# unslothai/unsloth

Measured on AMD Instinct MI355X. Metric: train tokens/sec, Llama-3-8B QLoRA (NF4) r=16 seq2048 bf16, higher is better.
Workload: dtype bf16; 1 GPU; Llama-3-8B QLoRA NF4 r=16 (q,k,v,o,gate,up,down) seq2048 bf16, fwd+bwd+AdamW; model=Llama-3-8B (synthetic weights), global_batch=4, seq_len=2048, parallelism=dp1, layers=32, lora_rank=16, gradient_checkpointing=unsloth, gc_schedule_chosen=all (every layer keeps everything), nf4_decoded_weight_mirrors=off (every NF4 weight is decoded at every use INSIDE the timed step), trainable_params=41943040, attention=csrc/attention.hip (causal GQA flash, fwd+bwd), optimizer=FlatAdamW fp32 on LoRA params

## Files before the change

include/unsloth_amd.h:

```cpp
#ifndef UNSLOTH_AMD_H
#define UNSLOTH_AMD_H

#include <stdint.h>

#ifdef __cplusplus
extern "C" {
#endif

#define UAMD_OK 0
#define UAMD_ERR_DTYPE (-1)
#define UAMD_ERR_ARG (-2)
#define UAMD_ERR_ALIGN (-3)

#define UAMD_F32 0
#define UAMD_F16 1
#define UAMD_BF16 2

int uamd_version(void);

int uamd_rms_layernorm_fwd(const void* X, const void* W, void* Y, float* r, int64_t n_rows,
                           int n_cols, int64_t x_row_stride, int64_t y_row_stride, float eps,
                           int gemma, int x_dtype, int w_dtype, void* stream);
int uamd_rms_layernorm_bwd(const void* dY, void* dX, const void* X, const void* W, const float* r,
                           int64_t n_rows, int n_cols, int64_t dy_row_stride,
// ... 14 lines not shown

int uamd_layernorm_fwd(const void* X, const void* W, const void* B, void* Y, float* r, float* mu, int64_t n_rows,
                       int n_cols, int64_t x_row_stride, int64_t y_row_stride, float eps, int x_dtype, int w_dtype,
                       void* stream);
int uamd_layernorm_bwd(void* dY, const void* X, const void* W, const float* r, const float* mu, int64_t n_rows,
                       int n_cols, int64_t dy_row_stride, int64_t x_row_stride, int x_dtype, int w_dtype, void* stream);

int uamd_rope_embedding(void* Q, int64_t q_row_stride, const void* cos, int64_t cos_row_stride,
                        const void* sin, int64_t sin_row_stride, int64_t n_rows, int seqlen,
                        int n_heads, int head_dim, int backward, int q_dtype, int table_dtype,
                        void* stream);
int uamd_rope_embedding_qk(void* Q, int64_t q_batch_stride, int64_t q_head_stride,
                           int64_t q_seq_stride, void* K, int64_t k_batch_stride,
                           int64_t k_head_stride, int64_t k_seq_stride, const void* cos,
                           int64_t cos_row_stride, const void* sin, int64_t sin_row_stride,
                           const int32_t* rope_indices, int batch, int seqlen, int n_heads_q,
                           int n_heads_k, int head_dim, int backward, int q_dtype,
                           int table_dtype, void* stream);

int uamd_rope_embedding_qk_mrope(void* Q, int64_t q_batch_stride, int64_t q_head_stride,
                                 int64_t q_seq_stride, void* K, int64_t k_batch_stride,
                                 int64_t k_head_stride, int64_t k_seq_stride, const void* cos,
                                 int64_t cos_row_stride, const void* sin, int64_t sin_row_stride,
                                 const int32_t* positions3, int section_t, int section_h, int batch,
                                 int seqlen, int n_heads_q, int n_heads_k, int head_dim, int backward,
                                 int q_dtype, int table_dtype, void* stream);

int uamd_swiglu_fg(const void* e, const void* g, void* h, int64_t n, int dtype, void* stream);
int uamd_swiglu_DWf_DW_dfg(void* DW, void* e, void* g, int64_t n, int dtype, void* stream);
int uamd_geglu_exact_forward(const void* e, const void* g, void* h, int64_t n, int dtype, void* stream);
int uamd_geglu_exact_backward(void* DW, void* e, void* g, int64_t n, int dtype, void* stream);
int uamd_geglu_approx_forward(const void* e, const void* g, void* h, int64_t n, int dtype, void* stream);
int uamd_geglu_approx_backward(void* DW, void* e, void* g, int64_t n, int dtype, void* stream);
int uamd_quick_gelu_forward(const void* x, void* y, int64_t n, int dtype, void* stream);
int uamd_quick_gelu_backward(const void* x, void* dy_dx, int64_t n, int dtype, void* stream);
int uamd_glu_fwd_xa(int act, const void* e, const void* g, void* h, int M, int K, int64_t ld, const void* W, int64_t ldw,
                    int R, float* out, int64_t ld_out, int out_cols, void* out_k, int64_t ld_k, int k_cols, int dtype,
                    void* stream);
int uamd_glu_bwd_xa(int act, void* DW, void* e, void* g, int M, int K, int64_t ld,
                    const void* Wu, int64_t ldwu, int Ru, float* out_u, int64_t ld_out_u, int out_cols_u,
                    void* out_k_u, int64_t ld_k_u, int k_cols_u,
                    const void* Wg, int64_t ldwg, int Rg, float* out_g, int64_t ld_out_g, int out_cols_g,
                    void* out_k_g, int64_t ld_k_g, int k_cols_g, int dtype, void* stream);
int64_t uamd_glu_xa_workspace(int M, int K, int n_products, int max_rank);
int uamd_glu_fwd_xa_ws(int act, const void* e, const void* g, void* h, int M, int K, int64_t ld, const void* W, int64_t ldw,
                       int R, float* out, int64_t ld_out, int out_cols, void* out_k, int64_t ld_k, int k_cols,
                       float* ws, int64_t ws_floats, int* counters, int dtype, void* stream);
int uamd_glu_bwd_xa_ws(int act, void* DW, void* e, void* g, int M, int K, int64_t ld,
                       const void* Wu, int64_t ldwu, int Ru, float* out_u, int64_t ld_out_u, int out_cols_u,
                       void* out_k_u, int64_t ld_k_u, int k_cols_u,
                       const void* Wg, int64_t ldwg, int Rg, float* out_g, int64_t ld_out_g, int out_cols_g,
                       void* out_k_g, int64_t ld_k_g, int k_cols_g, float* ws, int64_t ws_floats, int* counters,
                       int dtype, void* stream);

int uamd_cross_entropy_forward(const void* logits, int64_t logits_row_stride, float* loss,
                               float* logsumexp, const int64_t* labels, int64_t n_rows,
                               int vocab_size, float logit_softcapping, float logit_scaling,
                               int dtype, void* stream);
int uamd_cross_entropy_backward(void* logits, int64_t logits_row_stride, const float* dloss,
                                int64_t dloss_stride, const float* logsumexp,
                                const int64_t* labels, int64_t n_rows, int vocab_size,
                                float logit_softcapping, float logit_scaling, int dtype,
                                void* stream);
int uamd_logprob_entropy_forward(const void* logits, int64_t logits_row_stride, float* logprob, float* logsumexp,
                                 float* entropy, const int64_t* index, int64_t n_rows, int vocab_size,
                                 float logit_softcapping, float logit_scaling, int dtype, void* stream);

void cdequantize_blockwise_fp32(float* code, unsigned char* A, float* absmax, float* out,
                                int blocksize, const int n, void* stream);
void cdequantize_blockwise_bf16_nf4(float* code, unsigned char* A, float* absmax, void* out,
                                    int blocksize, const int n, void* stream);
void cdequantize_blockwise_fp16_nf4(float* code, unsigned char* A, float* absmax, void* out,
                                    int blocksize, const int n, void* stream);
void cdequantize_blockwise_fp32_nf4(float* code, unsigned char* A, float* absmax, void* out,
                                    int blocksize, const int n, void* stream);

int uamd_dequantize_absmax(const float* code2, const uint8_t* absmax_u8, const float* absmax2,
                           float offset, float* out, int blocksize2, int64_t n, void* stream);
int uamd_nf4_dequantize(const uint8_t* packed, const float* absmax_f32, const uint8_t* absmax_u8,
                        const float* code2, const float* absmax2, float offset, int blocksize2,
                        const float* nf4_lut, void* out, int64_t rows, int64_t cols, int blocksize,
                        int out_dtype, int transpose_out, int64_t ld_out, void* stream);
int uamd_nf4_dequantize_multi(int nseg, const uint8_t* const* packed, const float* const* absmax_f32,
                              void* const* out, const int64_t* numel, const float* const* nf4_lut, int blocksize,
                              int out_dtype, void* stream);
int uamd_nf4_quantize(const void* in, uint8_t* packed, float* absmax, int64_t n, int blocksize,
                      int in_dtype, void* stream);

typedef struct {
    const void* B;
    void* C;
    const float* absmax;
    const float* lora_xa;
    const void* lora_b;
    int64_t ldb, ldc, ld_xa, ld_lb;
    int N;
    int R;
    float lora_scale;
    int _pad;
    const void* lora_xk;
    const void* lora_bk;
    int64_t ld_xk, ld_bk;
    int Rk;
    int _pad2;
    const void* bias;
} uamd_gemm_group;
// ... 142 lines not shown
```

unsloth_amd/_lib.py:

```python
import ctypes
import os
from contextlib import nullcontext

import torch

c_void_p, c_int, c_int64, c_float = ctypes.c_void_p, ctypes.c_int, ctypes.c_int64, ctypes.c_float

HERE = os.path.dirname(os.path.abspath(__file__))
LIB_PATH = os.environ.get("UNSLOTH_AMD_LIB") or os.path.join(HERE, "lib", "libunsloth_amd.so")

UAMD_F32, UAMD_F16, UAMD_BF16 = 0, 1, 2
_DTYPE_CODE = {torch.float32: UAMD_F32, torch.float16: UAMD_F16, torch.bfloat16: UAMD_BF16}
_ERR = {-1: "unsupported dtype", -2: "invalid argument", -3: "pointer/stride not 16-byte aligned"}


class GemmGroup(ctypes.Structure):

    _fields_ = [
        ("B", c_void_p), ("C", c_void_p), ("absmax", c_void_p), ("lora_xa", c_void_p),
        ("lora_b", c_void_p), ("ldb", c_int64), ("ldc", c_int64), ("ld_xa", c_int64),
        ("ld_lb", c_int64), ("N", c_int), ("R", c_int), ("lora_scale", c_float), ("_pad", c_int),
        ("lora_xk", c_void_p), ("lora_bk", c_void_p), ("ld_xk", c_int64), ("ld_bk", c_int64), ("Rk", c_int),
        ("_pad2", c_int), ("bias", c_void_p),
    ]
# ... 56 lines not shown
    "uamd_quick_gelu_backward": (c_int, [c_void_p, c_void_p, c_int64, c_int, c_void_p]),
    "uamd_cross_entropy_forward": (c_int, [c_void_p, c_int64, c_void_p, c_void_p, c_void_p, c_int64,
                                           c_int, c_float, c_float, c_int, c_void_p]),
    "uamd_cross_entropy_backward": (c_int, [c_void_p, c_int64, c_void_p, c_int64, c_void_p, c_void_p,
                                            c_int64, c_int, c_float, c_float, c_int, c_void_p]),
    "uamd_logprob_entropy_forward": (c_int, [c_void_p, c_int64, c_void_p, c_void_p, c_void_p, c_void_p, c_int64,
                                             c_int, c_float, c_float, c_int, c_void_p]),
    "cdequantize_blockwise_fp32": (None, [c_void_p, c_void_p, c_void_p, c_void_p, c_int, c_int, c_void_p]),
    "cdequantize_blockwise_bf16_nf4": (None, [c_void_p, c_void_p, c_void_p, c_void_p, c_int, c_int, c_void_p]),
    "cdequantize_blockwise_fp16_nf4": (None, [c_void_p, c_void_p, c_void_p, c_void_p, c_int, c_int, c_void_p]),
    "cdequantize_blockwise_fp32_nf4": (None, [c_void_p, c_void_p, c_void_p, c_void_p, c_int, c_int, c_void_p]),
    "uamd_dequantize_absmax": (c_int, [c_void_p, c_void_p, c_void_p, c_float, c_void_p, c_int, c_int64,
                                       c_void_p]),
    "uamd_nf4_dequantize": (c_int, [c_void_p, c_void_p, c_void_p, c_void_p, c_void_p, c_float, c_int,
                                    c_void_p, c_void_p, c_int64, c_int64, c_int, c_int, c_int, c_int64,
                                    c_void_p]),
    "uamd_nf4_dequantize_multi": (c_int, [c_int, ctypes.POINTER(c_void_p), ctypes.POINTER(c_void_p), ctypes.POINTER(c_void_p),
                                          ctypes.POINTER(c_int64), ctypes.POINTER(c_void_p), c_int, c_int, c_void_p]),
    "uamd_nf4_quantize": (c_int, [c_void_p, c_void_p, c_void_p, c_int64, c_int, c_int, c_void_p]),
    "uamd_gemm_nt": (c_int, [c_void_p, c_int64, c_int, c_int, ctypes.POINTER(GemmGroup), c_int, c_int,
                             c_int, c_void_p]),
    "uamd_gemm_nt_256": (c_int, [c_void_p, c_int64, c_int, c_int, ctypes.POINTER(GemmGroup), c_int, c_int,
                                 c_int, c_void_p]),
    "uamd_gemm_nn_256": (c_int, [c_void_p, c_int64, c_int, c_int, ctypes.POINTER(GemmGroup), c_int, c_int,
                                 c_int, c_void_p]),
    "uamd_gemm_tn_256": (c_int, [c_void_p, c_int64, c_int, c_int, ctypes.POINTER(GemmGroup), c_int, c_int,
                                 c_int, c_void_p]),
    "uamd_set_tuning": (c_int, [c_int, c_int]),
    "uamd_gemm_nt_nf4": (c_int, [c_void_p, c_int64, c_int, c_int, ctypes.POINTER(GemmGroup), c_int,
                                 c_int, c_int, c_void_p]),
    "uamd_lora_xa": (c_int, [c_void_p, c_int64, c_void_p, c_int64, c_void_p, c_int64, c_int, c_int,
                             c_int, c_int, c_int, c_void_p]),
    "uamd_lora_xa2": (c_int, [c_void_p, c_int64, c_void_p, c_int64, c_void_p, c_int64, c_int, c_int,
                              c_int, c_int, c_int, c_void_p]),
    "uamd_lora_xa2k": (c_int, [c_void_p, c_int64, c_void_p, c_int64, c_void_p, c_int64, c_void_p, c_int64, c_int,
                               c_int, c_int, c_int, c_int, c_int, c_void_p]),
    "uamd_add_rms_layernorm_fwd": (c_int, [c_void_p] * 6 + [c_int64, c_int, c_int64, c_int64, c_int64, c_int64, c_float,
                                                             c_int, c_int, c_void_p]),
    "uamd_add_rms_layernorm_bwd": (c_int, [c_void_p] * 6 + [c_int64, c_int, c_int64, c_int64, c_int64, c_int64, c_int,
                                                             c_int, c_void_p]),
    "uamd_lora_prepare": (c_int, [c_void_p, c_void_p, c_int, c_int, c_int, c_void_p]),
    "uamd_adamw_flat": (c_int, [c_void_p, c_void_p, c_void_p, c_void_p, c_int64] + [ctypes.c_double] * 8 + [c_int, c_void_p]),
    "uamd_glu_fwd_xa": (c_int, [c_int, c_void_p, c_void_p, c_void_p, c_int, c_int, c_int64, c_void_p, c_int64, c_int,
                                c_void_p, c_int64, c_int, c_void_p, c_int64, c_int, c_int, c_void_p]),
    "uamd_glu_bwd_xa": (c_int, [c_int, c_void_p, c_void_p, c_void_p, c_int, c_int, c_int64]
                        + [c_void_p, c_int64, c_int, c_void_p, c_int64, c_int, c_void_p, c_int64, c_int] * 2
                        + [c_int, c_void_p]),
    "uamd_glu_xa_workspace": (c_int64, [c_int, c_int, c_int, c_int]),
    "uamd_glu_fwd_xa_ws": (c_int, [c_int, c_void_p, c_void_p, c_void_p, c_int, c_int, c_int64, c_void_p, c_int64, c_int,
                                   c_void_p, c_int64, c_int, c_void_p, c_int64, c_int, c_void_p, c_int64, c_void_p, c_int, c_void_p]),
    "uamd_glu_bwd_xa_ws": (c_int, [c_int, c_void_p, c_void_p, c_void_p, c_int, c_int, c_int64]
                           + [c_void_p, c_int64, c_int, c_void_p, c_int64, c_int, c_void_p, c_int64, c_int] * 2
                           + [c_void_p, c_int64, c_void_p, c_int, c_void_p]),
    "uamd_adamw_shard": (c_int, [c_void_p, c_void_p, c_void_p, c_void_p, c_void_p, c_int64] + [ctypes.c_double] * 8
                         + [c_int, c_void_p]),
    "uamd_adamw8_flat": (c_int, [c_void_p] * 8 + [c_int64] + [ctypes.c_double] * 8 + [c_int, c_void_p]),
    "uamd_adamw8_shard": (c_int, [c_void_p] * 9 + [c_int64] * 3 + [ctypes.c_double] * 8 + [c_int, c_void_p]),
    "uamd_lora_tn": (c_int, [ctypes.POINTER(LoraTnProblem), c_int, c_int, c_void_p, c_int64, c_int, c_void_p]),
    "uamd_attn_fwd": (c_int, [c_void_p, c_void_p, c_void_p, c_void_p, c_void_p, ctypes.POINTER(c_int64), c_int, c_int,
                              c_int, c_int, c_int, c_int, c_float, c_int, c_void_p, c_int, c_void_p]),
    "uamd_attn_fwd_band": (c_int, [c_void_p, c_void_p, c_void_p, c_void_p, c_void_p, ctypes.POINTER(c_int64), c_int, c_int,
                                   c_int, c_int, c_int, c_int, c_float, c_int, c_void_p, c_void_p, c_int, c_void_p]),
    "uamd_attn_bwd": (c_int, [c_void_p] * 10 + [ctypes.POINTER(c_int64), c_int, c_int, c_int, c_int, c_int, c_int,
                                               c_float, c_int, c_void_p, c_void_p, c_int, c_void_p]),
    "uamd_gemv": (c_int, [c_void_p, c_int, ctypes.POINTER(GemvGroup), c_int, c_int, c_int, c_int, c_void_p]),
    "uamd_gemv_fused": (c_int, [c_void_p, c_int, ctypes.POINTER(GemvGroup), c_int, c_int, c_int, c_int, c_void_p,
                                ctypes.POINTER(GemvPrologue)]),
    "uamd_rope_kv_append": (c_int, [c_void_p, c_int64, c_void_p, c_void_p, c_int64, c_void_p, c_void_p, c_void_p, c_void_p,
                                    c_int64, c_int64, c_int, c_int, c_int, c_int, c_int, c_int, c_void_p]),
    "uamd_attn_decode": (c_int, [c_void_p, c_int64, c_void_p, c_void_p, c_int64, c_int64, c_void_p, c_int, c_void_p,
                                 c_void_p, c_int64, c_int, c_int, c_int, c_int, c_int, c_int, c_int, c_float, c_int,
                                 c_void_p]),
    "uamd_attn_decode_fused": (c_int, [c_void_p, c_int64, c_void_p, c_void_p, c_int64, c_void_p, c_void_p, c_void_p, c_void_p,
                                       c_int64, c_int64, c_void_p, c_void_p, c_void_p, c_int64, c_int, c_int, c_int, c_int,
                                       c_int, c_int, c_int, c_int, c_float, ctypes.c_uint, c_void_p, c_int, c_void_p]),
    "uamd_argmax_f32": (c_int, [c_void_p, c_int, c_int64, c_void_p, c_void_p, c_void_p, c_void_p]),
    "uamd_debug_mfma_probe": (c_int, [c_void_p, c_void_p]),
}

_LIB = None


def lib():
    global _LIB
    if _LIB is None:
        if not os.path.exists(LIB_PATH):
            raise RuntimeError(
                f"unsloth_amd: {LIB_PATH} is missing. Build it with `python -m unsloth_amd._build` "
                "(hipcc, gfx950). There is no CPU / PyTorch fallback for the fused kernels."
            )
        handle = ctypes.CDLL(LIB_PATH)
        for name, (res, args) in SIGNATURES.items():
            fn = getattr(handle, name)
            fn.restype = res
            fn.argtypes = args
        _LIB = handle
    return _LIB


def dtype_code(dtype):
    try:
        return _DTYPE_CODE[dtype]
    except KeyError:
        raise TypeError(f"unsloth_amd kernels support fp32/fp16/bf16, got {dtype}") from None


# ... 38 lines not shown
```

unsloth_amd/csrc/glu.hip:

```cpp
#include "common.h"

namespace {

enum { ACT_SWIGLU = 0, ACT_GEGLU_EXACT = 1, ACT_GEGLU_APPROX = 2 };

__device__ __forceinline__ float sigmoidf_(float x) { return uamd_sigmoid(x); }

template <int ACT>
__device__ __forceinline__ void act_fwd(float e, float& f) {
    if (ACT == ACT_SWIGLU) {
        f = e * sigmoidf_(e);
    } else if (ACT == ACT_GEGLU_EXACT) {
        f = 0.5f * e * (erff(0.70710678118654752440f * e) + 1.0f);
    } else {
        const float s = 0.7978845608028654f;
        f = 0.5f * e * (tanhf(s * e * (1.0f + 0.044715f * e * e)) + 1.0f);
    }
}

template <int ACT>
__device__ __forceinline__ void act_bwd(float e, float& f, float& dfde) {
    if (ACT == ACT_SWIGLU) {
        const float se = sigmoidf_(e);
        f = se * e;
// ... 469 lines not shown
    if (rc) return rc;
    if (NS > 1 && (rc = check_xa_out(o1))) return rc;
    hipStream_t st = (hipStream_t)stream;
    if (ws != nullptr && ws_floats < xa_ws_floats(M, K, NS, NS > 1 ? (o0.R > o1.R ? o0.R : o1.R) : o0.R)) return UAMD_ERR_ARG;
    UAMD_DISPATCH_HALF(dtype,
        if (act == ACT_SWIGLU) return launch_xa<T, ACT_SWIGLU, NS>(dw, e, g, h, M, K, ld, o0, o1, st, ws, counters);
        if (act == ACT_GEGLU_EXACT) return launch_xa<T, ACT_GEGLU_EXACT, NS>(dw, e, g, h, M, K, ld, o0, o1, st, ws, counters);
        if (act == ACT_GEGLU_APPROX) return launch_xa<T, ACT_GEGLU_APPROX, NS>(dw, e, g, h, M, K, ld, o0, o1, st, ws, counters);
        return UAMD_ERR_ARG)
    return UAMD_ERR_DTYPE;
}

}

extern "C" int uamd_glu_fwd_xa(int act, const void* e, const void* g, void* h, int M, int K, int64_t ld, const void* W,
                               int64_t ldw, int R, float* out, int64_t ld_out, int out_cols, void* out_k, int64_t ld_k,
                               int k_cols, int dtype, void* stream) {
    return uamd_glu_fwd_xa_ws(act, e, g, h, M, K, ld, W, ldw, R, out, ld_out, out_cols, out_k, ld_k, k_cols, nullptr, 0, nullptr,
                              dtype, stream);
}

extern "C" int uamd_glu_bwd_xa(int act, void* DW, void* e, void* g, int M, int K, int64_t ld,
                               const void* Wu, int64_t ldwu, int Ru, float* out_u, int64_t ld_out_u, int out_cols_u,
                               void* out_k_u, int64_t ld_k_u, int k_cols_u,
                               const void* Wg, int64_t ldwg, int Rg, float* out_g, int64_t ld_out_g, int out_cols_g,
                               void* out_k_g, int64_t ld_k_g, int k_cols_g, int dtype, void* stream) {
    return uamd_glu_bwd_xa_ws(act, DW, e, g, M, K, ld, Wu, ldwu, Ru, out_u, ld_out_u, out_cols_u, out_k_u, ld_k_u, k_cols_u,
                              Wg, ldwg, Rg, out_g, ld_out_g, out_cols_g, out_k_g, ld_k_g, k_cols_g, nullptr, 0, nullptr, dtype, stream);
}

extern "C" int64_t uamd_glu_xa_workspace(int M, int K, int n_products, int max_rank) {
    if (M < 0 || K <= 0 || n_products < 1 || n_products > 2 || max_rank < 1 || max_rank > 64) return -1;
    return xa_ws_floats(M, K, n_products, max_rank);
}
extern "C" int uamd_glu_fwd_xa_ws(int act, const void* e, const void* g, void* h, int M, int K, int64_t ld, const void* W,
                                  int64_t ldw, int R, float* out, int64_t ld_out, int out_cols, void* out_k, int64_t ld_k,
                                  int k_cols, float* ws, int64_t ws_floats, int* counters, int dtype, void* stream) {
    GluXaOut o0{out, ld_out, R, out_cols, out_k, ld_k, k_cols, W, ldw};
    return glu_xa_entry<1>(act, nullptr, const_cast<void*>(e), const_cast<void*>(g), h, M, K, ld, o0, o0, dtype, stream, ws,
                           ws_floats, counters);
}
extern "C" int uamd_glu_bwd_xa_ws(int act, void* DW, void* e, void* g, int M, int K, int64_t ld,
                                  const void* Wu, int64_t ldwu, int Ru, float* out_u, int64_t ld_out_u, int out_cols_u,
                                  void* out_k_u, int64_t ld_k_u, int k_cols_u,
                                  const void* Wg, int64_t ldwg, int Rg, float* out_g, int64_t ld_out_g, int out_cols_g,
                                  void* out_k_g, int64_t ld_k_g, int k_cols_g, float* ws, int64_t ws_floats, int* counters,
                                  int dtype, void* stream) {
    GluXaOut o0{out_u, ld_out_u, Ru, out_cols_u, out_k_u, ld_k_u, k_cols_u, Wu, ldwu};
    GluXaOut o1{out_g, ld_out_g, Rg, out_cols_g, out_k_g, ld_k_g, k_cols_g, Wg, ldwg};
    return glu_xa_entry<2>(act, DW, e, g, nullptr, M, K, ld, o0, o1, dtype, stream, ws, ws_floats, counters);
}

namespace {
template <typename T, bool BWD>
__global__ void __launch_bounds__(256) quick_gelu_kernel(const T* __restrict__ X, T* __restrict__ Y, int64_t n) {
    constexpr int VEC = Vec16<T>::N;
    const int64_t nvec = n / VEC;
    for (int64_t i = (int64_t)blockIdx.x * 256 + threadIdx.x; i < nvec; i += (int64_t)gridDim.x * 256) {
        Vec16<T> x = ld16_m(X + i * VEC, 0), y;
        if (BWD) y = ld16_m(Y + i * VEC, 0);
#pragma unroll
        for (int j = 0; j < VEC; ++j) {
            const float v = to_f32(x.e[j]);
            const float sg = uamd_sigmoid(1.702f * v);
            if (BWD) y.e[j] = from_f32<T>(to_f32(y.e[j]) * (sg + 1.702f * v * sg * (1.0f - sg)));
            else y.e[j] = from_f32<T>(v * sg);
        }
        st16_m(Y + i * VEC, y, 0);
    }
    if (blockIdx.x == 0) {
        for (int64_t k = nvec * VEC + threadIdx.x; k < n; k += 256) {
            const float v = to_f32(X[k]);
            const float sg = uamd_sigmoid(1.702f * v);
            Y[k] = from_f32<T>(BWD ? to_f32(Y[k]) * (sg + 1.702f * v * sg * (1.0f - sg)) : v * sg);
        }
    }
}
template <typename T, bool BWD>
int launch_quick_gelu(const void* x, void* y, int64_t n, hipStream_t st) {
    if (!aligned16(x) || !aligned16(y)) return UAMD_ERR_ALIGN;
    const int64_t nvec = n / Vec16<T>::N;
    int64_t blocks = (nvec + 255) / 256;
    if (blocks < 1) blocks = 1;
    if (blocks > 256 * 16) blocks = 256 * 16;
    hipLaunchKernelGGL((quick_gelu_kernel<T, BWD>), dim3((unsigned)blocks), dim3(256), 0, st, (const T*)x, (T*)y, n);
    return uamd_launch_status();
}
}

extern "C" int uamd_quick_gelu_forward(const void* x, void* y, int64_t n, int dtype, void* stream) {
    if (n < 0 || (n > 0 && (!x || !y))) return UAMD_ERR_ARG;
    if (n == 0) return UAMD_OK;
    UAMD_DISPATCH_FLOAT(dtype, return (launch_quick_gelu<T, false>(x, y, n, (hipStream_t)stream)))
    return UAMD_ERR_DTYPE;
}
extern "C" int uamd_quick_gelu_backward(const void* x, void* dy_dx, int64_t n, int dtype, void* stream) {
    if (n < 0 || (n > 0 && (!x || !dy_dx))) return UAMD_ERR_ARG;
    if (n == 0) return UAMD_OK;
    UAMD_DISPATCH_FLOAT(dtype, return (launch_quick_gelu<T, true>(x, dy_dx, n, (hipStream_t)stream)))
    return UAMD_ERR_DTYPE;
}

extern "C" int uamd_swiglu_fg(const void* e, const void* g, void* h, int64_t n, int dtype, void* stream) {
    return glu<ACT_SWIGLU, false>(const_cast<void*>(e), const_cast<void*>(g), h, n, dtype, stream);
}
extern "C" int uamd_swiglu_DWf_DW_dfg(void* DW, void* e, void* g, int64_t n, int dtype, void* stream) {
// ... 15 lines not shown
```

unsloth_amd/kernels/fast_lora.py:

```python
import os

import torch

from .utils import _same_rows, alloc_rows, glu_bwd_terms, glu_fwd_xa
from .utils import (
    GRAD_SINKS,
    grad_sink,
    cast_lora,
    get_lora_parameters,
    lora_dx_terms,
    lora_linear_dx,
    lora_linear_forward,
    lora_tn,
    lora_tn_supported,
)
from .swiglu import swiglu_fg_kernel, swiglu_DWf_DW_dfg_kernel
from .geglu import (
    geglu_exact_forward_kernel,
    geglu_exact_backward_kernel,
    geglu_approx_forward_kernel,
    geglu_approx_backward_kernel,
)

try:
    _custom_fwd = torch.amp.custom_fwd(device_type="cuda")
    _custom_bwd = torch.amp.custom_bwd(device_type="cuda")
except Exception:
    _custom_fwd = lambda f: f
    _custom_bwd = lambda f: f


def _lora_grads(X2d, dY2d, A, B, s, dtype):
    if A is None:
        return None, None
    At, Bt = cast_lora(A, dtype).t(), cast_lora(B, dtype).t()
    dA_t = torch.empty_like(At)
    dB_t = torch.empty_like(Bt)
    dA_t.addmm_(X2d.t(), dY2d @ Bt.t(), alpha=s, beta=0)
    dB_t.addmm_(At.t() @ X2d.t(), dY2d, alpha=s, beta=0)
    return dA_t.t(), dB_t.t()


def _lora_grads_fused(items):
    probs, slots, targets, sinks = [], [], [], []
    for (X2d, dY2d, A, B, s, XA, P) in items:
        if A is None:
            slots.append(None)
            continue
        r = A.shape[0]
        slots.append(len(probs))
        probs.append((P, X2d, r, False, s))
        probs.append((XA, dY2d, r, True, s))
        for prm in (A, B):
            sink = grad_sink(prm)
            sinks.append((sink, prm))
            targets.append(sink.grad_view(prm) if sink is not None else None)
    outs = lora_tn(probs, targets if any(t is not None for t in targets) else None)
    for sink, prm in sinks:
        if sink is not None:
            sink.ready(prm)
    outs = [None if sk[0] is not None else o for o, sk in zip(outs, sinks)]
    return [(None, None) if k is None else (outs[k], outs[k + 1]) for k in slots]


_ACT_NAMES = {swiglu_fg_kernel: "swiglu", swiglu_DWf_DW_dfg_kernel: "swiglu",
              geglu_exact_forward_kernel: "geglu_exact", geglu_exact_backward_kernel: "geglu_exact",
              geglu_approx_forward_kernel: "geglu_approx", geglu_approx_backward_kernel: "geglu_approx"}


def _gate_up(X, gate, up, return_xa=False):
    outs = None
    widths = [(q.shape[0] if q is not None else W.shape[0]) for (W, q, *_rest) in (gate, up)]
    if (X.is_cuda and X.dtype in (torch.bfloat16, torch.float16) and widths[0] == widths[1]
            and widths[0] % 64 == 0 and all(len(p) <= 5 or p[5] is None for p in (gate, up))):
        M = X.numel() // X.shape[-1]
        eg = alloc_rows(M, 2 * widths[0], X.dtype, X.device)
        outs = [eg[:, :widths[0]], eg[:, widths[0]:]]
    return lora_linear_forward(X, [gate, up], outs=outs, return_xa=return_xa)


def mlp_forward(X, gate, up, down, act_fwd):
    (e, g), xa_gu = _gate_up(X, gate, up, return_xa=True)
    act = _ACT_NAMES.get(act_fwd)
    e2, g2 = e.view(-1, e.shape[-1]), g.view(-1, g.shape[-1])
    fused = glu_fwd_xa(act, e2, g2, down) if (act is not None and _same_rows([e2, g2])) else None
    if fused is not None:
        h, pre = fused
        (out,), xa_d = lora_linear_forward(h.view(e.shape), [down], return_xa=True, pre_xa=pre)
    else:
        if not e.is_contiguous():
            e, g = e.contiguous(), g.contiguous()
        h = act_fwd(e, g)
        (out,), xa_d = lora_linear_forward(h, [down], return_xa=True)
    return out, e, g, (xa_gu[0], xa_gu[1], xa_d[0])


def mlp_gate_up_forward(X, gate, up):
    return _gate_up(X, gate, up)


def mlp_backward(dY, X, e, g, xas, gate, up, down, act_bwd, inplace=True):
    xa_g, xa_u, xa_d = xas
    shape = X.shape
    dY = dY.reshape(-1, dY.shape[-1])
    X2 = X.reshape(-1, X.shape[-1])
    e = e.view(-1, e.shape[-1])
    g = g.view(-1, g.shape[-1])
    dtype = X2.dtype
    (p_d,) = lora_dx_terms([dY], [down])
    padded = e.stride(0) != e.shape[1] and _same_rows([e, g])
    DW = lora_linear_dx([dY], [down], terms=[p_d],
                        out=alloc_rows(e.shape[0], e.shape[1], e.dtype, e.device, ld=e.stride(0)) if padded else None)
    act = _ACT_NAMES.get(act_bwd)
    fused = glu_bwd_terms(act, DW, e, g, up, gate) if (act is not None and DW.dim() == 2) else None
    if fused is not None:
        h, df, de, (p_u, p_g) = fused
    else:
        if padded:
            DW, e, g = DW.contiguous(), e.contiguous(), g.contiguous()
        DW, e, g = act_bwd(DW, e, g)
        h, df, de = DW, e, g
        p_u, p_g = lora_dx_terms([df, de], [up, gate])
    if lora_tn_supported([h, dY, X2, df, de]):
        (d_downA, d_downB), (d_upA, d_upB), (d_gateA, d_gateB) = _lora_grads_fused([
            (h, dY, down[2], down[3], down[4], xa_d, p_d), (X2, df, up[2], up[3], up[4], xa_u, p_u),
            (X2, de, gate[2], gate[3], gate[4], xa_g, p_g)])
    else:
        d_downA, d_downB = _lora_grads(h, dY, down[2], down[3], down[4], dtype)
        d_upA, d_upB = _lora_grads(X2, df, up[2], up[3], up[4], dtype)
        d_gateA, d_gateB = _lora_grads(X2, de, gate[2], gate[3], gate[4], dtype)
    dX = lora_linear_dx([df, de], [up, gate], out=X2 if (inplace and X2.is_contiguous()) else None, terms=[p_u, p_g])
    return dX.view(shape), (d_gateA, d_gateB, d_upA, d_upB, d_downA, d_downB)


def qkv_forward(X, q, k, v):
    (Q, K, V), xa = lora_linear_forward(X, [q, k, v], return_xa=True)
    return Q, K, V, tuple(xa)


def qkv_backward(dQ, dK, dV, X, xas, q, k, v, inplace=True):
    xa_q, xa_k, xa_v = xas
    shape = X.shape
    dQ = dQ.reshape(-1, dQ.shape[-1])
    dK = dK.reshape(-1, dK.shape[-1])
    dV = dV.reshape(-1, dV.shape[-1])
    X2 = X.reshape(-1, X.shape[-1])
    projs = [q, k, v]
    p_q, p_k, p_v = lora_dx_terms([dQ, dK, dV], projs)
    if lora_tn_supported([X2, dQ, dK, dV]):
        (d_QA, d_QB), (d_KA, d_KB), (d_VA, d_VB) = _lora_grads_fused([
            (X2, dQ, q[2], q[3], q[4], xa_q, p_q), (X2, dK, k[2], k[3], k[4], xa_k, p_k),
            (X2, dV, v[2], v[3], v[4], xa_v, p_v)])
    else:
        d_QA, d_QB = _lora_grads(X2, dQ, q[2], q[3], q[4], X2.dtype)
        d_KA, d_KB = _lora_grads(X2, dK, k[2], k[3], k[4], X2.dtype)
        d_VA, d_VB = _lora_grads(X2, dV, v[2], v[3], v[4], X2.dtype)
    dX = lora_linear_dx([dQ, dK, dV], projs, out=X2 if (inplace and X2.is_contiguous()) else None,
                        terms=[p_q, p_k, p_v])
    return dX.view(shape), (d_QA, d_QB, d_KA, d_KB, d_VA, d_VB)


def w_forward(X, proj):
    (XW,), xa = lora_linear_forward(X, [proj], return_xa=True)
    return XW, xa[0]


# ... 139 lines not shown
```

unsloth_amd/kernels/utils.py:

```python
import ctypes
import os

import torch

from .. import _lib
from .. import nf4 as _nf4
from .._lib import GemmGroup

MAX_FUSED_SIZE = 65536
next_power_of_2 = lambda n: 1 << (max(int(n), 1) - 1).bit_length()

FUSED_NF4 = True
FUSED_NF4_MAX_M = 512
GEMM256_MODE = "auto"
GEMM256_MIN_TILES = 160
LORA_XA_V2 = True


def calculate_settings(n):
    BLOCK_SIZE = next_power_of_2(n)
    num_warps = 4
    if BLOCK_SIZE >= 32768:
        num_warps = 32
    elif BLOCK_SIZE >= 8192:
# ... 839 lines not shown
    r = A.shape[0]
    W, q = down[0], down[1]
    N = q.shape[0] if q is not None else W.shape[0]
    want_k = (not _fused_nf4(q, M, K)) and _use_gemm256(M, K, [N])
    Ac = cast_lora(A, dtype)
    h = alloc_rows(M, K, dtype, e.device, ld=e.stride(0))
    xa = torch.empty((M, r), dtype=torch.float32, device=e.device)
    xk = torch.empty((M, _rank_width(r)), dtype=dtype, device=e.device) if want_k else None
    with _lib.device_ctx(e):
        part, counters = _glu_workspace(e, 1, r)
        rc = _lib.lib().uamd_glu_fwd_xa_ws(_GLU_ACTS[act], _lib.ptr(e), _lib.ptr(g), _lib.ptr(h), M, K, e.stride(0), _lib.ptr(Ac),
                                           Ac.stride(0), r, _lib.ptr(xa), xa.stride(0), r,
                                           _lib.ptr(xk) if xk is not None else None, xk.stride(0) if xk is not None else 0,
                                           xk.shape[1] if xk is not None else 0, _lib.ptr(part), part.numel(), _lib.ptr(counters),
                                           _lib.dtype_code(dtype), _lib.stream_of(e))
    if rc != 0:
        counters.zero_()
    _lib.check(rc, "uamd_glu_fwd_xa_ws")
    return h, (xa, [(0, r)], xk)


def glu_bwd_terms(act, DW, e, g, up, gate):
    (Au, Bu), (Ag, Bg) = (up[2], up[3]), (gate[2], gate[3])
    if act != "swiglu" or Au is None or Ag is None or not _glu_fusable(e.dtype, [DW, e, g], [Au.shape[0], Ag.shape[0]], True):
        return None
    M, K = e.shape
    dtype = e.dtype
    ru, rg = Au.shape[0], Ag.shape[0]
    Kin = [(p[1].shape[1] if p[1] is not None else p[0].shape[1]) for p in (up, gate)]
    want_k = all(_use_gemm256(M, 64, [k]) for k in Kin)
    But, Bgt = cast_lora_t(Bu, dtype), cast_lora_t(Bg, dtype)
    shared = torch.empty((M, ru + rg), dtype=torch.float32, device=e.device)
    xk = torch.empty((M, _rank_width(ru + rg)), dtype=dtype, device=e.device) if want_k else None
    pu, pg = shared[:, :ru], shared[:, ru:]
    null = None
    with _lib.device_ctx(e):
        part, counters = _glu_workspace(e, 2, max(ru, rg))
        rc = _lib.lib().uamd_glu_bwd_xa_ws(
            _GLU_ACTS[act], _lib.ptr(DW), _lib.ptr(e), _lib.ptr(g), M, K, e.stride(0),
            _lib.ptr(But), But.stride(0), ru, _lib.ptr(pu), shared.stride(0), ru,
            _lib.ptr(xk) if want_k else null, xk.stride(0) if want_k else 0, ru if want_k else 0,
            _lib.ptr(Bgt), Bgt.stride(0), rg, _lib.ptr(pg), shared.stride(0), rg,
            _lib.ptr(xk[:, ru:]) if want_k else null, xk.stride(0) if want_k else 0, (xk.shape[1] - ru) if want_k else 0,
            _lib.ptr(part), part.numel(), _lib.ptr(counters), _lib.dtype_code(dtype), _lib.stream_of(e))
    if rc != 0:
        counters.zero_()
    _lib.check(rc, "uamd_glu_bwd_xa_ws")
    if want_k:
        pu._uamd_xk = (xk, 0)
        pg._uamd_xk = (xk, ru)
    return DW, e, g, [pu, pg]


def dense_dw(dY, X, out=None, accumulate=False):
    dY2d, X2d = _rows2d(dY), _rows2d(X)
    _lib.require_gpu(X2d)
    T, N_out = dY2d.shape
    assert X2d.shape[0] == T and X2d.dtype == dY2d.dtype
    dtype = X2d.dtype
    if dtype not in (torch.bfloat16, torch.float16):
        raise NotImplementedError("the MFMA GEMM path takes bf16/fp16 activations")
    N_in = X2d.shape[1]
    if N_out % 8 or N_in % 8:
        raise NotImplementedError(f"dense_dw: out {N_out} / in {N_in} features must be multiples of 8")
    if T % 64:
        pad = 64 - T % 64
        dY2d = torch.nn.functional.pad(dY2d, (0, 0, 0, pad))
        X2d = torch.nn.functional.pad(X2d, (0, 0, 0, pad))
        T += pad
    if out is None:
        out = torch.empty((N_out, N_in), dtype=dtype, device=X2d.device)
        accumulate = False
    if out.dtype != dtype or tuple(out.shape) != (N_out, N_in) or out.stride(1) != 1:
        raise ValueError(f"dense_dw: out must be a {dtype} [{N_out}, {N_in}] matrix of unit column stride, got {out.dtype} "
                         f"{tuple(out.shape)} with strides {out.stride()}")
    item = X2d.element_size()
    for t0, rows in _row_spans(T, max(dY2d.stride(0), X2d.stride(0)) * item, 64):
        g = _group(X2d, out, N_in, X2d.stride(0))
        g.B += t0 * X2d.stride(0) * item
        _lib.call("uamd_gemm_tn_256", X2d, ctypes.c_void_p(dY2d.data_ptr() + t0 * dY2d.stride(0) * item), dY2d.stride(0),
                  N_out, rows, (GemmGroup * 1)(g), 1, int(bool(accumulate) or t0 > 0), _lib.dtype_code(dtype),
                  _lib.stream_of(X2d))
    return out


def matmul_lora(X, W, W_quant, A, B, s, out=None):
    reshape = X.dim() == 3
    if reshape:
        batch, seq_len, _ = X.shape
    transposed = (W_quant is not None and W.shape[0] == 1) or (
        W_quant is None and W.dim() == 2 and W.stride(0) == 1 and W.stride(1) != 1)
    if not transposed:
        res = lora_linear_forward(X, [(W, W_quant, A, B, s)], outs=None if out is None else [out])[0]
    else:
        Wn = W.t()
        proj = (Wn, W_quant, None if B is None else B.t(), None if A is None else A.t(), s)
        res = lora_linear_dx([X], [proj], out=out)
    return res.view(batch, seq_len, -1) if reshape else res


def fast_linear_forward(proj, X, temp_lora=None, out=None):
    from . import decode as _dk
    W, W_quant, A, B, s, bias = get_lora_parameters_bias(proj)
    _refuse_fp8([(W,)])
    bsz, q_len, in_dim = X.shape
    n_out = int(W_quant.shape[0]) if W_quant is not None else int(W.shape[0])
# ... 21 lines not shown
```

Baseline: 35920 tokens/s.

## Fuse SwiGLU backward with LoRA weight-gradient reductions in one MLP kernel

```diff
diff --git a/include/unsloth_amd.h b/include/unsloth_amd.h
--- a/include/unsloth_amd.h
+++ b/include/unsloth_amd.h
@@ -90,6 +90,13 @@
                        const void* Wg, int64_t ldwg, int Rg, float* out_g, int64_t ld_out_g, int out_cols_g,
                        void* out_k_g, int64_t ld_k_g, int k_cols_g, float* ws, int64_t ws_floats, int* counters,
                        int dtype, void* stream);
+int64_t uamd_glu_tn_workspace(int M, int K);
+int uamd_glu_bwd_tn_ws(const void* DW, void* e, void* g, int M, int K, int64_t ld,
+                       const void* Wu, int64_t ldwu, int Ru, const void* Wg, int64_t ldwg, int Rg,
+                       float* out_rows, int64_t ld_out, void* out_k, int64_t ld_k, int k_cols,
+                       const float* Pd, int64_t ldpd, int Rd, const float* Pu, int64_t ldpu, const float* Pg,
+                       int64_t ldpg, float* dA_down, float* dB_up, float* dB_gate, float s_down, float s_up,
+                       float s_gate, int accumulate, void* ws, int64_t ws_bytes, int dtype, void* stream);
 
 int uamd_cross_entropy_forward(const void* logits, int64_t logits_row_stride, float* loss,
                                float* logsumexp, const int64_t* labels, int64_t n_rows,
diff --git a/unsloth_amd/_lib.py b/unsloth_amd/_lib.py
--- a/unsloth_amd/_lib.py
+++ b/unsloth_amd/_lib.py
@@ -132,6 +132,11 @@
     "uamd_glu_bwd_xa_ws": (c_int, [c_int, c_void_p, c_void_p, c_void_p, c_int, c_int, c_int64]
                            + [c_void_p, c_int64, c_int, c_void_p, c_int64, c_int, c_void_p, c_int64, c_int] * 2
                            + [c_void_p, c_int64, c_void_p, c_int, c_void_p]),
+    "uamd_glu_tn_workspace": (c_int64, [c_int, c_int]),
+    "uamd_glu_bwd_tn_ws": (c_int, [c_void_p, c_void_p, c_void_p, c_int, c_int, c_int64]
+                           + [c_void_p, c_int64, c_int] * 2 + [c_void_p, c_int64, c_void_p, c_int64, c_int]
+                           + [c_void_p, c_int64, c_int, c_void_p, c_int64, c_void_p, c_int64]
+                           + [c_void_p] * 3 + [c_float] * 3 + [c_int, c_void_p, c_int64, c_int, c_void_p]),
     "uamd_adamw_shard": (c_int, [c_void_p, c_void_p, c_void_p, c_void_p, c_void_p, c_int64] + [ctypes.c_double] * 8
                          + [c_int, c_void_p]),
     "uamd_adamw8_flat": (c_int, [c_void_p] * 8 + [c_int64] + [ctypes.c_double] * 8 + [c_int, c_void_p]),
diff --git a/unsloth_amd/csrc/glu.hip b/unsloth_amd/csrc/glu.hip
--- a/unsloth_amd/csrc/glu.hip
+++ b/unsloth_amd/csrc/glu.hip
@@ -545,6 +545,324 @@
 }
 
 namespace {
+typedef __attribute__((ext_vector_type(4))) __bf16 glu_bf16x4_t;
+typedef __attribute__((ext_vector_type(4))) _Float16 glu_f16x4_t;
+typedef __attribute__((ext_vector_type(4))) short glu_s16x4_t;
+typedef __attribute__((address_space(3))) glu_s16x4_t glu_lds_s16x4;
+template <typename T> struct GluMfma16;
+template <> struct GluMfma16<bf16_t> {
+    typedef glu_bf16x4_t frag;
+    static __device__ __forceinline__ glu_f32x4_t run(frag a, frag b, glu_f32x4_t c) {
+        return __builtin_amdgcn_mfma_f32_16x16x16bf16_1k(a, b, c, 0, 0, 0);
+    }
+};
+template <> struct GluMfma16<f16_t> {
+    typedef glu_f16x4_t frag;
+    static __device__ __forceinline__ glu_f32x4_t run(frag a, frag b, glu_f32x4_t c) {
+        return __builtin_amdgcn_mfma_f32_16x16x16f16(a, b, c, 0, 0, 0);
+    }
+};
+
+#ifndef UAMD_GT_RPC_MAX
+#define UAMD_GT_RPC_MAX 512
+#endif
+#ifndef UAMD_GT_MIN_WGS
+#define UAMD_GT_MIN_WGS 512
+#endif
+constexpr int GT_PT = 4 * 16 * 16 * 2;
+constexpr int GT_RED = 8 * 16 * 16 * 4;
+constexpr int GT_BUF = 3 * GX_TILE + GT_PT + GT_RED;
+constexpr int GT_LDS = 2 * GT_BUF;
+
+struct GluTnArgs {
+    const void* DW;
+    void* E;
+    void* G;
+    int M, K;
+    int64_t ld;
+    const void* W[2];
+    int64_t ldw[2];
+    int Rw[2];
+    const float* P[3];
+    int64_t ldp[3];
+    int Rp[3];
+    int rpc, S, n_strips;
+    float* part_rows;
+    float* part_G;
+    float* out_rows;
+    int64_t ld_out;
+    void* out_k;
+    int64_t ld_k;
+    int k_cols;
+    float* grad[3];
+    float scale[3];
+    int accumulate;
+};
+
+template <typename T>
+__global__ void __launch_bounds__(512, 4) glu_tn_kernel(GluTnArgs a) {
+    extern __shared__ __attribute__((aligned(16))) unsigned char smem[];
+    typedef typename GluMfma<T>::frag frag_t;
+    typedef typename GluMfma16<T>::frag frag4_t;
+    const int tid = threadIdx.x, lane = tid & 63, wave = tid >> 6;
+    const int l15 = lane & 15, l4 = lane >> 4;
+    const int chunk = (int)(blockIdx.x / (unsigned)a.n_strips);
+    const int strip = (int)(blockIdx.x - (unsigned)chunk * (unsigned)a.n_strips);
+    const int M = a.M, K = a.K;
+    const int64_t ld = a.ld;
+    const T* DW = (const T*)a.DW;
+    T* E = (T*)a.E;
+    T* G = (T*)a.G;
+    const int m_base = chunk * a.rpc;
+    const int m_end = min(m_base + a.rpc, M);
+    const int ntiles = (m_end - m_base + 15) >> 4;
+    const int srow = tid >> 5, scol = (tid & 31) * 8;
+    const int c = strip * GX_TK + scol;
+    const bool col_ok = c + 8 <= K;
+    const int cc = col_ok ? c : 0;
+    const int pz = tid >> 7, prow = (tid & 127) >> 3, prank = (tid & 7) * 2;
+    const int pzz = pz < 3 ? pz : 0;
+    const float* Pz = pzz == 1 ? a.P[1] : pzz == 2 ? a.P[2] : a.P[0];
+    const int64_t ldp = pzz == 1 ? a.ldp[1] : pzz == 2 ? a.ldp[2] : a.ldp[0];
+    const int Rp = pzz == 1 ? a.Rp[1] : pzz == 2 ? a.Rp[2] : a.Rp[0];
+    const bool rank_ok = prank + 2 <= Rp;
+    const int pcol = rank_ok ? prank : 0;
+    const int rp = wave & 1, ks0 = (wave >> 1) * 2;
+    uint4 wf[2];
+    {
+        const T* W = (const T*)a.W[rp];
+        const int64_t wo = (int64_t)min(l15, a.Rw[rp] - 1) * a.ldw[rp];
+#pragma unroll
+        for (int q = 0; q < 2; ++q) {
+            const int kc = strip * GX_TK + (ks0 + q) * 32 + l4 * 8;
+            wf[q] = kc + 8 <= K ? *reinterpret_cast<const uint4*>(W + wo + kc) : make_uint4(0, 0, 0, 0);
+        }
+    }
+    glu_f32x4_t acc[3][2];
+#pragma unroll
+    for (int z = 0; z < 3; ++z)
+#pragma unroll
+        for (int b = 0; b < 2; ++b) acc[z][b] = glu_f32x4_t{0.f, 0.f, 0.f, 0.f};
+    const int st_off = srow * GX_LD + scol * 2;
+    const int pt_off = 3 * GX_TILE + ((pz * 16 + prank) * 16 + prow) * 2;
+    const int pa_off = 3 * GX_TILE + (l15 * 16 + 4 * l4) * 2;
+    const int tr_off = (4 * l4 + (l15 >> 2)) * GX_LD + (wave * 32 + (l15 & 3) * 4) * 2;
+    const int ra_off = l15 * GX_LD + (ks0 * 32 + l4 * 8) * 2;
+    const int rw_off = 3 * GX_TILE + GT_PT + ((wave * 16 + 4 * l4) * 16 + l15) * 4;
+    const int er_off = 3 * GX_TILE + GT_PT + ((((tid >> 4) & 1) * 16 + srow) * 16 + (tid & 15)) * 4;
+    float* prow_out = a.part_rows + ((int64_t)strip * M) * 32 + (tid & 31);
+
+    struct Regs {
+        Vec16<T> e, g, dw;
+        float2 p;
+    };
+    Regs A, B;
+    auto load_tile = [&](int it, Regs& r) {
+        const int m0 = m_base + it * 16;
+        const int64_t o = (int64_t)min(m0 + srow, M - 1) * ld + cc;
+        r.e = ld16_nt(E + o);
+        r.g = ld16_nt(G + o);
+        r.dw = ld16_nt(DW + o);
+        r.p = *reinterpret_cast<const float2*>(Pz + (int64_t)min(m0 + prow, M - 1) * ldp + pcol);
+        __builtin_amdgcn_sched_barrier(0);
+    };
+    auto emit_rows = [&](int it) {
+        const float* q = reinterpret_cast<const float*>(smem + (it & 1) * GT_BUF + er_off);
+        const float v = ((q[0] + q[2 * 256]) + q[4 * 256]) + q[6 * 256];
+        const int m = m_base + it * 16 + srow;
+        if (m < M) prow_out[(int64_t)m * 32] = v;
+    };
+    auto tile = [&](int it, Regs& r, Regs& rn, int it_next, auto emit_prev) {
+        unsigned char* buf = smem + (it & 1) * GT_BUF;
+        load_tile(it_next, rn);
+        const int m0 = m_base + it * 16;
+        Vec16<T> h, v0, v1;
+#pragma unroll
+        for (int j = 0; j < 8; ++j) bwd_one<T, ACT_SWIGLU>(r.dw.e[j], r.e.e[j], r.g.e[j], h.e[j], v0.e[j], v1.e[j]);
+        if (col_ok && m0 + srow < M) {
+            const int64_t o = (int64_t)(m0 + srow) * ld + c;
+            st16_nt(E + o, v0);
+            st16_nt(G + o, v1);
+        }
+        if (!col_ok) {
+            h.raw = make_uint4(0, 0, 0, 0);
+            v0.raw = make_uint4(0, 0, 0, 0);
+            v1.raw = make_uint4(0, 0, 0, 0);
+        }
+        *reinterpret_cast<uint4*>(buf + st_off) = h.raw;
+        *reinterpret_cast<uint4*>(buf + st_off + GX_TILE) = v0.raw;
+        *reinterpret_cast<uint4*>(buf + st_off + 2 * GX_TILE) = v1.raw;
+        const bool p_ok = rank_ok && m0 + prow < M;
+        *reinterpret_cast<T*>(buf + pt_off) = from_f32<T>(p_ok ? r.p.x : 0.f);
+        *reinterpret_cast<T*>(buf + pt_off + 32) = from_f32<T>(p_ok ? r.p.y : 0.f);
+        asm volatile("s_waitcnt lgkmcnt(0)" ::: "memory");
+        __builtin_amdgcn_s_barrier();
+        asm volatile("" ::: "memory");
+        if constexpr (decltype(emit_prev)::value) emit_rows(it - 1);
+        union { uint2 r; frag4_t f; } pa[3];
+#pragma unroll
+        for (int z = 0; z < 3; ++z) pa[z].r = *reinterpret_cast<const uint2*>(buf + pa_off + z * 512);
+#pragma unroll
+        for (int b = 0; b < 2; ++b)
+#pragma unroll
+            for (int z = 0; z < 3; ++z) {
+                union { glu_s16x4_t h; frag4_t f; } zb;
+                zb.h = __builtin_amdgcn_ds_read_tr16_b64_v4i16((glu_lds_s16x4*)(buf + z * GX_TILE + tr_off + b * 32));
+                acc[z][b] = GluMfma16<T>::run(pa[z].f, zb.f, acc[z][b]);
+            }
+        glu_f32x4_t racc = glu_f32x4_t{0.f, 0.f, 0.f, 0.f};
+#pragma unroll
+        for (int q = 0; q < 2; ++q) {
+            union { uint4 r; frag_t f; } x, w;
+            x.r = *reinterpret_cast<const uint4*>(buf + (1 + rp) * GX_TILE + ra_off + q * 64);
+            w.r = wf[q];
+            racc = GluMfma<T>::run(x.f, w.f, racc);
+        }
+#pragma unroll
+        for (int i = 0; i < 4; ++i) *reinterpret_cast<float*>(buf + rw_off + i * 64) = racc[i];
+    };
+    constexpr std::true_type yes{};
+    constexpr std::false_type no{};
+    load_tile(0, A);
+    tile(0, A, B, ntiles > 1 ? 1 : 0, no);
+    int it = 1;
+    for (; it + 1 < ntiles; it += 2) {
+        tile(it, B, A, it + 1, yes);
+        tile(it + 1, A, B, it + 2 < ntiles ? it + 2 : it + 1, yes);
+    }
+    if (it < ntiles) tile(it, B, A, it, yes);
+    __syncthreads();
+    emit_rows(ntiles - 1);
+    const int64_t kpad = (int64_t)a.n_strips * GX_TK;
+    float* pg = a.part_G + ((int64_t)chunk * 3 * 16 + 4 * l4) * kpad + strip * GX_TK + wave * 32 + l15;
+#pragma unroll
+    for (int z = 0; z < 3; ++z)
+#pragma unroll
+        for (int b = 0; b < 2; ++b)
+#pragma unroll
+            for (int i = 0; i < 4; ++i) pg[((int64_t)z * 16 + i) * kpad + b * 16] = acc[z][b][i];
+}
+
+template <typename T>
+__global__ void __launch_bounds__(256) glu_tn_reduce_kernel(GluTnArgs a, int nb_rows) {
+    const int M = a.M, K = a.K;
+    const int Ru = a.Rw[0], Rg = a.Rw[1];
+    if ((int)blockIdx.x < nb_rows) {
+        const int64_t idx = (int64_t)blockIdx.x * 256 + threadIdx.x;
+        if (idx >= (int64_t)M * 32) return;
+        const int64_t m = idx >> 5;
+        const int cl = (int)(idx & 31), p = cl >> 4, rank = cl & 15;
+        const float* q = a.part_rows + idx;
+        const int64_t sstride = (int64_t)M * 32;
+        float v = 0.f;
+        int s = 0;
+        for (; s + 8 <= a.n_strips; s += 8) {
+            float t[8];
+#pragma unroll
+            for (int u = 0; u < 8; ++u) t[u] = q[(int64_t)(s + u) * sstride];
+#pragma unroll
+            for (int u = 0; u < 8; ++u) v += t[u];
+        }
+        for (; s < a.n_strips; ++s) v += q[(int64_t)s * sstride];
+        if (rank < (p ? Rg : Ru)) {
+            const int col = (p ? Ru : 0) + rank;
+            a.out_rows[m * a.ld_out + col] = v;
+            if (a.out_k != nullptr) ((T*)a.out_k)[m * a.ld_k + col] = from_f32<T>(v);
+        }
+        if (a.out_k != nullptr)
+            for (int cz = Ru + Rg + cl; cz < a.k_cols; cz += 32) ((T*)a.out_k)[m * a.ld_k + cz] = from_f32<T>(0.f);
+        return;
+    }
+    const int64_t idx = (int64_t)(blockIdx.x - nb_rows) * 256 + threadIdx.x;
+    if (idx >= (int64_t)48 * K) return;
+    const int zr = (int)(idx / K), n = (int)(idx - (int64_t)zr * K);
+    const int z = zr >> 4, r = zr & 15;
+    const int R = a.Rp[z];
+    if (r >= R) return;
+    const int64_t kpad = (int64_t)a.n_strips * GX_TK;
+    const float* q = a.part_G + (int64_t)zr * kpad + n;
+    const int64_t sstride = 48 * kpad;
+    float v = 0.f;
+    int s = 0;
+    for (; s + 8 <= a.S; s += 8) {
+        float t[8];
+#pragma unroll
+        for (int u = 0; u < 8; ++u) t[u] = q[(int64_t)(s + u) * sstride];
+#pragma unroll
+        for (int u = 0; u < 8; ++u) v += t[u];
+    }
+    for (; s < a.S; ++s) v += q[(int64_t)s * sstride];
+    v *= a.scale[z];
+    float* o = z == 0 ? a.grad[0] + (int64_t)r * K + n : a.grad[z] + (int64_t)n * R + r;
+    *o = ((a.accumulate >> z) & 1) ? *o + v : v;
+}
+
+inline void tn_plan(int M, int K, int& rpc, int& S, int& n_strips) {
+    n_strips = (K + GX_TK - 1) / GX_TK;
+    rpc = UAMD_GT_RPC_MAX;
+    while (rpc > 128 && (int64_t)n_strips * ((M + rpc - 1) / rpc) < UAMD_GT_MIN_WGS) rpc >>= 1;
+    S = (M + rpc - 1) / rpc;
+}
+inline int64_t tn_rows_floats(int M, int n_strips) { return (int64_t)n_strips * M * 32; }
+inline int64_t tn_grad_floats(int S, int n_strips) { return (int64_t)S * 48 * n_strips * GX_TK; }
+
+template <typename T>
+int launch_tn(GluTnArgs& a, hipStream_t st) {
+    const int64_t blocks = (int64_t)a.S * a.n_strips;
+    const int64_t nb_rows = ((int64_t)a.M * 32 + 255) / 256, nb_grad = ((int64_t)48 * a.K + 255) / 256;
+    if (blocks > 0x7fffffffLL || nb_rows + nb_grad > 0x7fffffffLL) return UAMD_ERR_ARG;
+    if (int rc = uamd_launch_lds<&glu_tn_kernel<T>>(dim3((unsigned)blocks), dim3(512), GT_LDS, st, a)) return rc;
+    hipLaunchKernelGGL((glu_tn_reduce_kernel<T>), dim3((unsigned)(nb_rows + nb_grad)), dim3(256), 0, st, a, (int)nb_rows);
+    return uamd_launch_status();
+}
+
+}
+
+extern "C" int64_t uamd_glu_tn_workspace(int M, int K) {
+    if (M < 0 || K < 8 || (K & 7)) return -1;
+    int rpc, S, n_strips;
+    tn_plan(M > 0 ? M : 1, K, rpc, S, n_strips);
+    return 4 * (tn_rows_floats(M, n_strips) + tn_grad_floats(S, n_strips));
+}
+
+extern "C" int uamd_glu_bwd_tn_ws(const void* DW, void* e, void* g, int M, int K, int64_t ld,
+                                  const void* Wu, int64_t ldwu, int Ru, const void* Wg, int64_t ldwg, int Rg,
+                                  float* out_rows, int64_t ld_out, void* out_k, int64_t ld_k, int k_cols,
+                                  const float* Pd, int64_t ldpd, int Rd, const float* Pu, int64_t ldpu, const float* Pg,
+                                  int64_t ldpg, float* dA_down, float* dB_up, float* dB_gate, float s_down, float s_up,
+                                  float s_gate, int accumulate, void* ws, int64_t ws_bytes, int dtype, void* stream) {
+    if (M < 0 || K < 8 || !DW || !e || !g || !Wu || !Wg || !out_rows || !Pd || !Pu || !Pg || !dA_down || !dB_up || !dB_gate || !ws)
+        return UAMD_ERR_ARG;
+    for (int R : {Ru, Rg, Rd})
+        if (R != 8 && R != 16) return UAMD_ERR_ARG;
+    if (ld < K || ldwu < K || ldwg < K || ld_out < Ru + Rg || ldpd < Rd || ldpu < Ru || ldpg < Rg) return UAMD_ERR_ARG;
+    if (out_k && (k_cols < Ru + Rg || ld_k < k_cols)) return UAMD_ERR_ARG;
+    if (M == 0) return UAMD_OK;
+    if ((K & 7) || (ld & 7) || (ldwu & 7) || (ldwg & 7) || !aligned16(DW) || !aligned16(e) || !aligned16(g) || !aligned16(Wu) ||
+        !aligned16(Wg))
+        return UAMD_ERR_ALIGN;
+    if ((ldpd & 1) || (ldpu & 1) || (ldpg & 1) || ((uintptr_t)Pd & 7) || ((uintptr_t)Pu & 7) || ((uintptr_t)Pg & 7) ||
+        ((uintptr_t)ws & 15))
+        return UAMD_ERR_ALIGN;
+    GluTnArgs a;
+    a.DW = DW; a.E = e; a.G = g; a.M = M; a.K = K; a.ld = ld;
+    a.W[0] = Wu; a.W[1] = Wg; a.ldw[0] = ldwu; a.ldw[1] = ldwg; a.Rw[0] = Ru; a.Rw[1] = Rg;
+    a.P[0] = Pd; a.P[1] = Pu; a.P[2] = Pg; a.ldp[0] = ldpd; a.ldp[1] = ldpu; a.ldp[2] = ldpg;
+    a.Rp[0] = Rd; a.Rp[1] = Ru; a.Rp[2] = Rg;
+    tn_plan(M, K, a.rpc, a.S, a.n_strips);
+    const int64_t rows_f = tn_rows_floats(M, a.n_strips);
+    if (ws_bytes < 4 * (rows_f + tn_grad_floats(a.S, a.n_strips))) return UAMD_ERR_ARG;
+    a.part_rows = (float*)ws;
+    a.part_G = (float*)ws + rows_f;
+    a.out_rows = out_rows; a.ld_out = ld_out; a.out_k = out_k; a.ld_k = ld_k; a.k_cols = out_k ? k_cols : 0;
+    a.grad[0] = dA_down; a.grad[1] = dB_up; a.grad[2] = dB_gate;
+    a.scale[0] = s_down; a.scale[1] = s_up; a.scale[2] = s_gate;
+    a.accumulate = accumulate;
+    UAMD_DISPATCH_HALF(dtype, return launch_tn<T>(a, (hipStream_t)stream))
+    return UAMD_ERR_DTYPE;
+}
+
+namespace {
 template <typename T, bool BWD>
 __global__ void __launch_bounds__(256) quick_gelu_kernel(const T* __restrict__ X, T* __restrict__ Y, int64_t n) {
     constexpr int VEC = Vec16<T>::N;
diff --git a/unsloth_amd/kernels/fast_lora.py b/unsloth_amd/kernels/fast_lora.py
--- a/unsloth_amd/kernels/fast_lora.py
+++ b/unsloth_amd/kernels/fast_lora.py
@@ -2,7 +2,7 @@
 
 import torch
 
-from .utils import _same_rows, alloc_rows, glu_bwd_terms, glu_fwd_xa
+from .utils import _same_rows, alloc_rows, glu_bwd_terms, glu_bwd_tn, glu_fwd_xa, glu_tn_takes
 from .utils import (
     GRAD_SINKS,
     grad_sink,
@@ -63,6 +63,26 @@
     return [(None, None) if k is None else (outs[k], outs[k + 1]) for k in slots]
 
 
+def _mlp_grads_tn(act, DW, e, g, dY, X2, xas, p_d, gate, up, down):
+    xa_g, xa_u, xa_d = xas
+    wide = [down[2], up[3], gate[3]]
+    narrow = [down[3], up[2], gate[2]]
+    sinks = [(grad_sink(prm), prm) for prm in wide + narrow]
+    targets = [sk.grad_view(prm) if sk is not None else None for sk, prm in sinks]
+    res = glu_bwd_tn(act, DW, e, g, up, gate, down, p_d, xa_u, xa_g, targets[:3])
+    if res is None:
+        return None
+    df, de, (p_u, p_g), outs = res
+    outs = outs + lora_tn([(xa_d, dY, down[2].shape[0], True, down[4]), (p_u, X2, up[2].shape[0], False, up[4]),
+                           (p_g, X2, gate[2].shape[0], False, gate[4])],
+                          targets[3:] if any(t is not None for t in targets[3:]) else None)
+    for sk, prm in sinks:
+        if sk is not None:
+            sk.ready(prm)
+    d_downA, d_upB, d_gateB, d_downB, d_upA, d_gateA = [None if sk[0] is not None else o for o, sk in zip(outs, sinks)]
+    return df, de, [p_u, p_g], (d_gateA, d_gateB, d_upA, d_upB, d_downA, d_downB)
+
+
 _ACT_NAMES = {swiglu_fg_kernel: "swiglu", swiglu_DWf_DW_dfg_kernel: "swiglu",
               geglu_exact_forward_kernel: "geglu_exact", geglu_exact_backward_kernel: "geglu_exact",
               geglu_approx_forward_kernel: "geglu_approx", geglu_approx_backward_kernel: "geglu_approx"}
@@ -112,6 +132,12 @@
     DW = lora_linear_dx([dY], [down], terms=[p_d],
                         out=alloc_rows(e.shape[0], e.shape[1], e.dtype, e.device, ld=e.stride(0)) if padded else None)
     act = _ACT_NAMES.get(act_bwd)
+    if act is not None and DW.dim() == 2 and glu_tn_takes(act, DW, e, g, up, gate, down) and lora_tn_supported([dY, X2]):
+        tn = _mlp_grads_tn(act, DW, e, g, dY, X2, xas, p_d, gate, up, down)
+        if tn is not None:
+            df, de, (p_u, p_g), grads = tn
+            dX = lora_linear_dx([df, de], [up, gate], out=X2 if (inplace and X2.is_contiguous()) else None, terms=[p_u, p_g])
+            return dX.view(shape), grads
     fused = glu_bwd_terms(act, DW, e, g, up, gate) if (act is not None and DW.dim() == 2) else None
     if fused is not None:
         h, df, de, (p_u, p_g) = fused
diff --git a/unsloth_amd/kernels/utils.py b/unsloth_amd/kernels/utils.py
--- a/unsloth_amd/kernels/utils.py
+++ b/unsloth_amd/kernels/utils.py
@@ -915,6 +915,69 @@
     return DW, e, g, [pu, pg]
 
 
+GLU_TN = True
+_GLU_TN_WS = {}
+
+
+def glu_tn_takes(act, DW, e, g, up, gate, down):
+    if not GLU_TN or act != "swiglu" or any(p[2] is None or p[3] is None for p in (up, gate, down)):
+        return False
+    ranks = [p[2].shape[0] for p in (up, gate, down)]
+    return (all(r <= 16 and r % 8 == 0 for r in ranks) and _glu_fusable(e.dtype, [DW, e, g], ranks, True)
+            and lora_tn_supported([DW, e, g]))
+
+
+def _tn_factor(P, R):
+    if P.dtype == torch.float32 and P.stride(1) == 1 and P.stride(0) % 2 == 0 and P.data_ptr() % 8 == 0:
+        return P
+    return P[:, :R].float().contiguous()
+
+
+def glu_bwd_tn(act, DW, e, g, up, gate, down, p_d, xa_u, xa_g, targets=None):
+    if not glu_tn_takes(act, DW, e, g, up, gate, down):
+        return None
+    M, K = e.shape
+    dtype, dev = e.dtype, e.device
+    ru, rg, rd = up[2].shape[0], gate[2].shape[0], down[2].shape[0]
+    if any(P.dim() != 2 or P.shape[0] != M or P.shape[1] < r for P, r in ((p_d, rd), (xa_u, ru), (xa_g, rg))):
+        raise ValueError("glu_bwd_tn: p_d / xa_u / xa_g must be fp32 [M, >= rank]")
+    Kin = [(p[1].shape[1] if p[1] is not None else p[0].shape[1]) for p in (up, gate)]
+    want_k = all(_use_gemm256(M, 64, [k]) for k in Kin)
+    But, Bgt = cast_lora_t(up[3], dtype), cast_lora_t(gate[3], dtype)
+    p_d, xa_u, xa_g = _tn_factor(p_d, rd), _tn_factor(xa_u, ru), _tn_factor(xa_g, rg)
+    shapes = [(rd, K), (K, ru), (K, rg)]
+    targets = list(targets) if targets is not None else [None] * 3
+    grads, acc = [], 0
+    for i, (tgt, shp) in enumerate(zip(targets, shapes)):
+        if tgt is not None:
+            assert tgt.dtype == torch.float32 and tgt.is_contiguous() and tgt.device == dev and tuple(tgt.shape) == shp
+            acc |= 1 << i
+        grads.append(tgt if tgt is not None else torch.empty(shp, dtype=torch.float32, device=dev))
+    shared = torch.empty((M, ru + rg), dtype=torch.float32, device=dev)
+    xk = torch.empty((M, _rank_width(ru + rg)), dtype=dtype, device=dev) if want_k else None
+    with _lib.device_ctx(e):
+        need = int(_lib.lib().uamd_glu_tn_workspace(M, K))
+        key = (dev.index, int(torch.cuda.current_stream(dev).cuda_stream))
+        ws = _GLU_TN_WS.get(key)
+        if need >= 0 and (ws is None or ws.numel() < need):
+            ws = _GLU_TN_WS[key] = torch.empty(need, dtype=torch.uint8, device=dev)
+        rc = -2 if need < 0 else _lib.lib().uamd_glu_bwd_tn_ws(
+            _lib.ptr(DW), _lib.ptr(e), _lib.ptr(g), M, K, e.stride(0),
+            _lib.ptr(But), But.stride(0), ru, _lib.ptr(Bgt), Bgt.stride(0), rg,
+            _lib.ptr(shared), shared.stride(0), _lib.ptr(xk), xk.stride(0) if want_k else 0, xk.shape[1] if want_k else 0,
+            _lib.ptr(p_d), p_d.stride(0), rd, _lib.ptr(xa_u), xa_u.stride(0), _lib.ptr(xa_g), xa_g.stride(0),
+            _lib.ptr(grads[0]), _lib.ptr(grads[1]), _lib.ptr(grads[2]), float(down[4]), float(up[4]), float(gate[4]), acc,
+            _lib.ptr(ws), ws.numel(), _lib.dtype_code(dtype), _lib.stream_of(e))
+    if rc in _lib._ERR:
+        return None
+    _lib.check(rc, "uamd_glu_bwd_tn_ws")
+    pu, pg = shared[:, :ru], shared[:, ru:]
+    if want_k:
+        pu._uamd_xk = (xk, 0)
+        pg._uamd_xk = (xk, ru)
+    return e, g, [pu, pg], grads
+
+
 def dense_dw(dY, X, out=None, accumulate=False):
     dY2d, X2d = _rows2d(dY), _rows2d(X)
     _lib.require_gpu(X2d)
```

Measured after the change: 36700 tokens/s (median of 6 runs). 2.2% higher.
